# dmiruke/find_motion

Measured on AMD Instinct MI355X. Metric: frames/sec on 1080p synthetic video at 1/2/4/8 MI355X; achieved HBM GB/s %peak, higher is better.
Workload: dtype u8+f64

## Files before the change

### find_motion_amd/csrc/fm_pix.hip

```cpp
#include <type_traits>

#include "fm_internal.h"

namespace fm {
namespace px {

constexpr int TS = 64;
constexpr int kPixWPE = 4;
constexpr int NT = 512;
constexpr int NW = NT / 64;
constexpr int RPWV = TS / NW;

__host__ __device__ constexpr int a16(int v) { return (v + 15) & ~15; }

struct Geo {
    int r, PC, GW, NQ, GH, RS, CPR, nchunks, RSH;
    int o_raw, o_H, o_rowy, o_colx, o_atab, bytes;
    int raw_bytes, H_bytes;
    __host__ __device__ explicit Geo(int rr) {
        r = rr;
        PC = 4 * ((r + 3) / 4);
        GW = TS + 2 * PC;
        NQ = GW / 4;
        GH = TS + 2 * r;
// ... 392 lines not shown
                    uint8_t* gp = a.planes + f * plane + (size_t)y * w;
#pragma unroll
                    for (int b = 0; b < 4; b++)
                        if (xq + b < w) gp[xq + b] = (uint8_t)(g4[it] >> (8 * b));
                }
            }
            uint32_t qv[NQW];
            qv[0] = g4[it];
#pragma unroll
            for (int d = 1; d < NQW; d++)
                qv[d] = d < NQN ? (uint32_t)__builtin_amdgcn_mov_dpp((int)qv[d - 1], 0x130, 0xF, 0xF, true) : 0u;
            {
                const uint32_t h0 = htap<0, OFF, NG, 0, NQW>(qv, cpk, 0u);
                const uint32_t h1 = htap<1, OFF, NG, 0, NQW>(qv, cpk, 0u);
                const uint32_t h2 = htap<2, OFF, NG, 0, NQW>(qv, cpk, 0u);
                const uint32_t h3 = htap<3, OFF, NG, 0, NQW>(qv, cpk, 0u);
                *reinterpret_cast<uint2*>(Hb + hoff[it]) = make_uint2(h0 | (h1 << 16), h2 | (h3 << 16));
            }
        }
    };
    auto stage_raw = [&](const Raw<NCH>& Rr, int buf) __attribute__((always_inline)) { store_raw(Rr, raw + buf * g.raw_bytes, g, tid); };

    const int t0 = a.t_begin, t1 = a.t_end;
    const int skip = __builtin_amdgcn_readfirstlane(a.dbg_skip);
    Raw<NCH> Rw;
    load_raw(Rw, a.src + ((size_t)t0 * S + s) * fbytes, fb32, plan, span);
    stage_raw(Rw, 0);
    if (t0 + 1 < t1) load_raw(Rw, a.src + ((size_t)(t0 + 1) * S + s) * fbytes, fb32, plan, span);
    lds_barrier();
    gray_stage(raw, Hs, (size_t)t0 * S + s);

    auto frame_loop = [&](auto keepc, auto tailc, const ChainCtx ccv) __attribute__((always_inline)) {
        constexpr bool KEEP = decltype(keepc)::value != 0, TAIL = decltype(tailc)::value != 0;
        for (int t = t0; t < t1; t++) {
            const int b = (t - t0) & 1;
            const size_t f = (size_t)t * S + s;
            if (t + 1 < t1) {
                if (!(skip & 8)) stage_raw(Rw, b ^ 1);
                if (t + 2 < t1 && !(skip & 4)) load_raw(Rw, a.src + (f + 2 * S) * fbytes, fb32, plan, span);
            }
            if (!(skip & 16)) lds_barrier();

            uint32_t colbits = 0;
            ChainCtx ccf = ccv;
            ccf.rowvalid = __builtin_amdgcn_readfirstlane(ccf.rowvalid);
            int x0f = __builtin_amdgcn_readfirstlane(x0), y0f = __builtin_amdgcn_readfirstlane(y0), wvf = wv;
            if constexpr (NT == 512) asm volatile("" : "+s"(ccf.colmask), "+s"(ccf.rowvalid), "+s"(x0f), "+s"(y0f), "+s"(wvf));
            asm volatile("" : "+v"(ccf.keep_lo), "+v"(ccf.keep_hi));
            if (!(skip & 2))
                chain_rows<KC, PLANES, INIT, KEEP, TAIL>(a, Hs + b * (g.H_bytes / 2), atab, g, bg, wvf, ln, x0f, y0f, f, ccf,
                                                         init0 && t == t0, colbits);
            reinterpret_cast<uint8_t*>(a.bits)[((f * a.ntiles + ti) * TS + ln) * 8 + wv] = (uint8_t)colbits;

            if (t + 1 < t1 && !(skip & 1))
                gray_stage(raw + (b ^ 1) * g.raw_bytes, Hs + (b ^ 1) * (g.H_bytes / 2), f + S);
        }
    };
    if (!cc.vec) frame_loop(IntC<1>{}, IntC<1>{}, cc);
    else if (cc.hk) frame_loop(IntC<1>{}, IntC<0>{}, cc);
    else frame_loop(IntC<0>{}, IntC<0>{}, cc);

    double* bgo = a.bg_out + (size_t)s * plane;
    const int x = x0 + ln;
#pragma unroll
    for (int j = 0; j < RPWV; j++) {
        const int y = y0 + RPWV * wv + j;
        if (x < w && y < h) bgo[(size_t)y * w + x] = bg[j];
    }
    kstamp_end(a.kstamp);
    if (pts) {
        const uint64_t rt = __builtin_amdgcn_s_memrealtime(), mt = __builtin_amdgcn_s_memtime();
        pts[1] = rt0;
        pts[2] = rt;
        pts[3] = mt - mt0;
    }
}

template <int K> constexpr int tap_c(int t) { return t < 0 || t >= K ? 0 : Taps<K>::c[t]; }
template <int K> constexpr int tap_lo() {
    int i = 0;
    while (Taps<K>::c[i] == 0) i++;
    return i;
}
template <int K> constexpr int tap_hi() {
    int i = K - 1;
    while (Taps<K>::c[i] == 0) i--;
    return i;
}

template <int KC, int RW_ = RPWV>
struct PW {
    static constexpr int NWB = 8;
    static constexpr int RW = RW_;
    static constexpr int R = KC / 2;
    static constexpr int PC = 4 * ((R + 3) / 4);
    static constexpr int NTB = 64 * NWB;
    static constexpr int TH = RW * NWB;
    static constexpr int GH = TH + 2 * R;
    static constexpr int GQ = (TS + 2 * PC) / 4;
    static constexpr int NG = GH * GQ;
    static constexpr int GSLOTS = (NG + 63) / 64;
    static constexpr int gcnt(int w) { return (GSLOTS - w + NWB - 1) / NWB; }
    static constexpr int GJ = gcnt(0);
    static constexpr int NHP = GH / 2;
    static constexpr int NH = NHP * (TS / 4);
    static constexpr int HJ = (NH + NTB - 1) / NTB;
    static constexpr int HLASTW = (NH - (HJ - 1) * NTB + 63) / 64;
#ifndef FM_PIXW_GS
#define FM_PIXW_GS 24
#endif
    static constexpr int GS = FM_PIXW_GS > GQ ? FM_PIXW_GS : GQ;
    static constexpr int GBUF = GH * GS + 64;
    static constexpr int HBUF = (NHP + 1) * TS;
    static constexpr int LO = tap_lo<KC>(), HI = tap_hi<KC>();
    static constexpr int NGR = (HI - LO + 4) / 4;
    static constexpr int OFF = PC - R;
    static constexpr int WQ = (3 + OFF + LO + 4 * NGR - 1) / 4 + 1;
    static constexpr int p0(int j) { return (j + LO) >> 1; }
    static constexpr int np(int j) { return (j + HI + 2 - 2 * p0(j)) / 2; }
    static constexpr int np_max() {
        int m = 0;
        for (int j = 0; j < RW; j++) m = p0(j) + np(j) > m ? p0(j) + np(j) : m;
        return m;
    }
    static constexpr int NP = np_max();
    static constexpr int bytes = 2 * GBUF * 4 + 2 * HBUF * 4 + 256 * 8;
    static constexpr int dyn_bytes = bytes - 256 * 8;
};
template <int KC> constexpr uint32_t tapw4(int g) {
    uint32_t v = 0;
    for (int b = 0; b < 4; b++) {
        const int t = PW<KC>::LO + 4 * g + b;
        if (t <= PW<KC>::HI) v |= (uint32_t)Taps<KC>::c[t] << (8 * b);
    }
    return v;
}
template <int KC> constexpr uint32_t tapv2(int j, int i) {
    const int ft = 2 * (PW<KC>::p0(j) + i) - j;
    return (uint32_t)tap_c<KC>(ft) | (uint32_t)tap_c<KC>(ft + 1) << 16;
}

template <int KC, int RW> constexpr int np_rows() {
    int m = 0;
    for (int j = 0; j < RW; j++) m = PW<KC>::p0(j) + PW<KC>::np(j) > m ? PW<KC>::p0(j) + PW<KC>::np(j) : m;
    return m;
}

template <int RW, int NPR>
__device__ __forceinline__ void chain_pairs(uint32_t (&P)[NPR], const uint32_t* Hp, int wv, int ln) {
    const uint32_t* col = Hp + (RW / 2 * wv) * TS + ln;
#pragma unroll
    for (int i = 0; i < NPR; i++) P[i] = col[i * TS];
}
template <int KC, bool KEEP, bool SDWA, int j, bool H16 = false, int NPR>
__device__ __forceinline__ void chain_blur(const uint32_t (&P)[NPR], const ChainCtx& cc, uint32_t& acc, uint32_t& tix) {
    using G = PW<KC>;
    acc = 32768u;
    static_for<G::np(j)>([&](auto ic) {
        constexpr int i = decltype(ic)::value;
        acc = __builtin_amdgcn_udot2(__builtin_bit_cast(u16x2_t, P[G::p0(j) + i]),
                                     __builtin_bit_cast(u16x2_t, tapv2<KC>(j, i) << (H16 ? 4 : 0)), acc, false);
    });
    if (KEEP) {
        const uint32_t kw = j < 4 ? cc.keep_lo : j < 8 ? cc.keep_hi : j < 12 ? cc.keep_2 : cc.keep_3;
        acc &= (uint32_t)__builtin_amdgcn_sbfe((int)kw, 8 * (j & 3), 8);
    }
    if constexpr (SDWA)
        asm("v_lshlrev_b32_sdwa %0, 3, %1 dst_sel:DWORD dst_unused:UNUSED_PAD src0_sel:DWORD src1_sel:BYTE_2"
            : "=v"(tix) : "v"(acc));
    else
        tix = acc >> 16;
}
template <bool SDWA>
__device__ __forceinline__ double chain_tab(const double* atab, uint32_t tix) {
    return SDWA ? *reinterpret_cast<const double*>(reinterpret_cast<const char*>(atab) + tix) : atab[tix];
}
template <int j>
__device__ __forceinline__ void chain_bit(uint32_t acc, double b, uint32_t bias, uint32_t& tb, uint32_t& tb2) {
    const uint32_t q = __builtin_amdgcn_cvt_pk_u8_f32(fabsf(__double2float_rn(b)), 2, acc);
    const uint32_t r = __builtin_amdgcn_sad_u8(acc, q, bias);
    if constexpr (j < 8) tb = __builtin_amdgcn_udot4(r, (1u << j) << 8, tb, false);
    else tb2 = __builtin_amdgcn_udot4(r, (1u << (j - 8)) << 8, tb2, false);
}
template <bool TAIL, int RW, int j>
__device__ __forceinline__ double chain_bg(const FusedArgs& a, double b, double beta, double bl, int wv, int ln, int x0, int y0,
                                           int w) {
    double nb = bg_fma(b, beta, bl);
    if (TAIL) {
        const long long li = (long long)(y0 + RW * wv + j) * w + x0 + ln;
        if (li >= a.acc_vec_end) nb = __dadd_rn(bl, __dmul_rn(b, beta));
    }
    return nb;
}
template <int RW>
__device__ __forceinline__ void chain_flags(uint32_t tb, uint32_t tb2, const ChainCtx& cc, uint32_t& colbits) {
    if constexpr (RW > 8) tb |= tb2 << 8;
    colbits = tb & cc.tbmask;
    asm volatile("" : "+v"(colbits));
}

template <int KC, bool KEEP, bool TAIL, bool SDWA, int RW = RPWV>
__device__ __forceinline__ void chain_rows_w(const FusedArgs& a, const uint32_t* Hp, const double* atab, double (&bg)[RW],
                                             int wv, int ln, int x0, int y0, const ChainCtx& cc, uint32_t& colbits) {
    static_assert(RW == 8 || RW == 16, "rows per wave");
    uint32_t P[np_rows<KC, RW>()];
    chain_pairs<RW>(P, Hp, wv, ln);
    const int w = a.w;
    const double beta = a.beta;
    const int thr = min(max(a.thresh, -1), 255);
    const uint32_t bias = (uint32_t)(255 - thr);
    uint32_t tb = 0, tb2 = 0;
    static_for<RW>([&](auto jc) {
        constexpr int j = decltype(jc)::value;
        uint32_t acc, tix;
        chain_blur<KC, KEEP, SDWA, j>(P, cc, acc, tix);
        const double b = bg[j];
        chain_bit<j>(acc, b, bias, tb, tb2);
        const double bl = chain_tab<SDWA>(atab, tix);
        bg[j] = chain_bg<TAIL, RW, j>(a, b, beta, bl, wv, ln, x0, y0, w);
    });
    chain_flags<RW>(tb, tb2, cc, colbits);
}

template <int K>
struct HS {
    static constexpr int LO = tap_lo<K>(), NTAPS = tap_hi<K>() - LO + 1, B0 = PW<K>::OFF + LO;
    static constexpr int d0(int k) { return (B0 + k) / 4; }
    static constexpr int nd(int k) { return (B0 + k + NTAPS - 1) / 4 - d0(k) + 1; }
    static constexpr int base(int k) { return k == 0 ? 0 : base(k - 1) + nd(k - 1); }
    static constexpr int NC = base(4);
    static constexpr int NQ = (B0 + 3 + NTAPS - 1) / 4 + 1;
    static constexpr uint32_t c(int k, int i) {
        uint32_t v = 0;
        const int d = d0(k) + i;
        for (int b = 0; b < 4; b++) {
            const int t = 4 * d + b - B0 - k;
            if (t >= 0 && t < NTAPS) v |= (uint32_t)Taps<K>::c[LO + t] << (8 * b);
        }
        return v;
    }
};
template <int K>
__device__ __forceinline__ void hs_consts(uint32_t (&cs)[HS<K>::NC]) {
    static_for<4>([&](auto kc) {
        constexpr int k = decltype(kc)::value;
        static_for<HS<K>::nd(k)>([&](auto ic) {
            constexpr int i = decltype(ic)::value;
            cs[HS<K>::base(k) + i] = HS<K>::c(k, i);
        });
    });
#pragma unroll
    for (int i = 0; i < HS<K>::NC; i++) asm volatile("" : "+v"(cs[i]));
}
template <int K, int k, int N>
__device__ __forceinline__ uint32_t hs_tap(const uint32_t (&q)[N], const uint32_t (&cs)[HS<K>::NC]) {
    static_assert(HS<K>::d0(k) + HS<K>::nd(k) <= N, "window dwords");
    uint32_t acc = 0;
    static_for<HS<K>::nd(k)>([&](auto ic) {
        constexpr int i = decltype(ic)::value;
        acc = __builtin_amdgcn_udot4(q[HS<K>::d0(k) + i], cs[HS<K>::base(k) + i], acc, false);
    });
    return acc;
}

template <int NWB_ = 8>
struct P5G {
    static constexpr int NWB = NWB_;
    static constexpr int RW = TS / NWB;
    static constexpr int NTB = 64 * NWB;
    static constexpr int TH = RW * NWB;
    static constexpr int GH = TH + 4;
    static constexpr int GQ = 18;
#ifndef FM_P5_GS
#define FM_P5_GS 24
#endif
#ifndef FM_P5_GS8
#define FM_P5_GS8 20
#endif
    static constexpr int GS = NWB == 8 ? FM_P5_GS8 : FM_P5_GS > GQ ? FM_P5_GS : GQ;
    static_assert(GS >= 20 && GS % 2 == 0, "a 32-byte window at byte 48 of an 8-byte aligned row");
    static constexpr int NG = GH * GQ;
    static constexpr int GSLOTS = (NG + 63) / 64;
    static constexpr int GFAST = NWB == 8 ? 4 : (GSLOTS + NWB - 1) / NWB;
    static constexpr int GSLOW = NWB == 8 ? (GSLOTS - 4 * GFAST + 3) / 4 : 0;
    static constexpr int GJ = GFAST > GSLOW ? GFAST : GSLOW;
    static constexpr int NH = (GH / 2) * (TS / 4);
    static constexpr int HJ = (NH + NTB - 1) / NTB;
    static constexpr int HLASTW = (NH - (HJ - 1) * NTB + 63) / 64;
    static constexpr int GBUF = GH * GS + 64;
    static constexpr int HBUF = (GH + 2) * TS;
    static constexpr int bytes = 2 * GBUF * 4 + 2 * HBUF * 2 + 256 * 8;
    static constexpr int dyn_bytes = bytes - 256 * 8;
    static constexpr int MROWS = GH / 2, MB = 3;
    static constexpr int moff(int i) { return i == 0 ? 0 : i == 1 ? 16 : MROWS - 16; }
};
static_assert(P5G<8>::MROWS % 2 == 0 && P5G<8>::moff(2) % 2 == 0 && P5G<8>::moff(2) <= 32, "whole row pairs, no gap");
static_assert(P5G<8>::GSLOW >= 0 && 4 * (P5G<8>::GFAST + P5G<8>::GSLOW) >= P5G<8>::GSLOTS, "gray slots");
static_assert(4 * P5G<4>::GFAST >= P5G<4>::GSLOTS, "gray slots");

template <int GJ>
struct P5Raw {
    u32x3_t v[GJ];
};

template <bool KEEP, bool TAIL, int NWB = 8>
__global__ __launch_bounds__(64 * NWB) __attribute__((amdgpu_waves_per_eu(kPixWPE))) void k_pix5(FusedArgs a) {
    using G = P5G<NWB>;
    constexpr int RW = G::RW;
    constexpr int GJX = G::GJ, HJX = G::HJ;
    extern __shared__ __attribute__((aligned(16))) uint8_t smem[];
    constexpr int KC = 5, R = 2;
    uint32_t* gray = reinterpret_cast<uint32_t*>(smem);
    uint16_t* Hs = reinterpret_cast<uint16_t*>(smem + 2 * G::GBUF * 4);
    __shared__ double atab_s[256];
    double* atab = atab_s;
    const int tid = (int)threadIdx.x, ln = tid & 63;
    const int wv = __builtin_amdgcn_readfirstlane(tid >> 6);
    const int s = blockIdx.y;
    const int h = a.h, w = a.w, S = a.S;
    const int ti = swizzle_tile(blockIdx.x, a.ntiles);
    const int tx = ti % a.ntx;
    const int y0 = (ti / a.ntx) * TS;
    const int x0 = tx * TS;
    const size_t plane = (size_t)h * w;
    const size_t fbytes = plane * 3;
    const bool hk = a.has_keep[s] != 0;
    const uint8_t* keep = a.keep + (size_t)s * plane;
    if (tid < 256) atab[tid] = __dmul_rn((double)tid, a.alpha);
    kstamp_begin(a.kstamp);
#ifdef FM_DEV_SWITCHES
    uint64_t* pts = (a.dbg_pts && tid == 0) ? a.dbg_pts + ((size_t)s * a.ntiles + ti) * 4 : nullptr;
    uint64_t rt0 = 0, mt0 = 0;
    if (pts) {
        pts[0] = (uint64_t)__builtin_amdgcn_s_getreg((31 << 11) | 4) | ((uint64_t)__builtin_amdgcn_s_getreg((31 << 11) | 20) << 32);
        rt0 = __builtin_amdgcn_s_memrealtime();
        mt0 = __builtin_amdgcn_s_memtime();
    }
#endif

    uint32_t goff[GJX];
    uint32_t gdst[GJX];
    const int gjobs = NWB == 8 ? (wv < 4 ? G::GFAST : G::GSLOW) : min(G::GFAST, G::GSLOTS - wv * G::GFAST);
#pragma unroll
    for (int i = 0; i < GJX; i++) {
        const int slot = NWB != 8 ? wv * G::GFAST + i : wv >= 4 ? (wv - 4) * G::GSLOW + i : 4 * G::GSLOW + wv * G::GFAST + i;
        const int j = i < gjobs ? slot * 64 + ln : G::NG;
        const int gr = j / G::GQ, gq = j - gr * G::GQ;
        const int x = x0 - 4 + 4 * gq;
        const bool live = j < G::NG && x >= 0 && x + 4 <= w;
        const int y = reflect101(y0 - R + gr, h);
        goff[i] = live ? (uint32_t)(((size_t)y * w + x) * 3) : 0u;
        gdst[i] = j < G::NG ? (uint32_t)(G::GS == G::GQ ? j : gr * G::GS + gq) : (uint32_t)(G::GH * G::GS + ln);
    }
    uint32_t hsrc[HJX], hdst[HJX];
#pragma unroll
    for (int i = 0; i < HJX; i++) {
        const int j = tid + G::NTB * i;
        const bool live = j < G::NH;
        const int hr = live ? j / (TS / 4) : 0, hq = live ? j - hr * (TS / 4) : 0;
        hsrc[i] = (uint32_t)(2 * hr * G::GS + hq);
        hdst[i] = (uint32_t)((live ? hr : G::GH / 2) * TS + 4 * hq);
    }
    const bool edge_tile = x0 == 0 || x0 + TS + 4 > w;
    const int vq = (w - x0 + 4) / 4;
    uint32_t hfix[HJX];
#pragma unroll
    for (int i = 0; i < HJX; i++) {
        const int hq = (int)(hsrc[i] % G::GS);
        hfix[i] = (x0 == 0 && hq == 0 ? 1u : 0u) | (hq + 1 == vq ? 2u : 0u) | (hq + 2 == vq ? 4u : 0u);
    }
    uint32_t asrc = 0, mdst = 0;
    long btap = 0;
    i32x4_t mc0 = {2048, 2048, 2048, 2048};
    if constexpr (NWB == 8) {
        static_assert(Taps<5>::c[0] % 16 == 0 && Taps<5>::c[1] % 16 == 0 && Taps<5>::c[2] % 16 == 0, "taps / 16");
        const int mn = ln & 15, mq = ln >> 4, cb = wv & 3, r0 = (wv >> 2) * G::MROWS;
        asrc = (uint32_t)((r0 + mn) * G::GS * 4 + 16 * cb + 8 * mq);
        mdst = (uint32_t)((r0 / 2 + 2 * mq) * TS + 16 * cb + mn);
        const int bw = w - x0 + 4;
        uint64_t bt = 0;
        static_for<5>([&](auto tc) {
            constexpr int t = decltype(tc)::value;
            int sb = 16 * cb + mn + 2 + t;
            if (x0 == 0 && sb < 4) sb = 8 - sb;
            else if (sb >= bw) sb = 2 * bw - 2 - sb;
            const int k = sb - 16 * cb - 8 * mq;
            bt += (unsigned)k < 8u ? (uint64_t)(Taps<5>::c[t] / 16) << (8 * (k & 7)) : 0ull;
        });
        btap = (long)bt;
        asm volatile("" : "+v"(asrc), "+v"(mdst), "+v"(btap), "+v"(mc0));
    }

    double bg[RW];
    ChainCtx cc;
    auto load_bg = [&]() __attribute__((always_inline)) {
        const double* bgi = a.bg_in + (size_t)s * plane;
        const int x = x0 + ln;
        cc.colmask = __builtin_amdgcn_ballot_w64(x < w);
        cc.rowvalid = 0;
        cc.keep_lo = cc.keep_hi = cc.keep_2 = cc.keep_3 = 0;
        cc.hk = __builtin_amdgcn_readfirstlane(hk ? 1 : 0) != 0;
#pragma unroll
        for (int j = 0; j < RW; j++) {
            const int y = y0 + RW * wv + j;
            const bool in = x < w && y < h;
            if (y < h) cc.rowvalid |= 1u << j;
            bg[j] = in ? bgi[(size_t)y * w + x] : 0.0;
            const uint32_t kb = (!hk || (in && keep[(size_t)y * w + x] != 0)) ? 0xFFu : 0u;
            if (j < 4) cc.keep_lo |= kb << (8 * j);
            else if (j < 8) cc.keep_hi |= kb << (8 * (j - 4));
            else if (j < 12) cc.keep_2 |= kb << (8 * (j - 8));
            else cc.keep_3 |= kb << (8 * (j - 12));
        }
        const long long last = (long long)(y0 + RW * wv + RW - 1) * w + x0 + TS - 1;
        cc.vec = (uint32_t)__builtin_amdgcn_readfirstlane(last < a.acc_vec_end ? 1 : 0);
        cc.tbmask = x < w ? cc.rowvalid : 0u;
#pragma unroll
        for (int j = 0; j < RW; j++) asm volatile("" : "+v"(bg[j]));
        asm volatile("" : "+v"(cc.keep_lo), "+v"(cc.keep_hi));
        if constexpr (RW > 8) asm volatile("" : "+v"(cc.keep_2), "+v"(cc.keep_3));
    };
    if constexpr (NWB != 8) load_bg();

    uint32_t hcs[HS<KC>::NC] = {};
    if constexpr (NWB != 8) hs_consts<KC>(hcs);
    P5Raw<GJX> rw;
    auto load = [&](size_t f) __attribute__((always_inline)) {
        const gbytes_t src = frame_base(a.src + f * fbytes);
#pragma unroll
        for (int i = 0; i < GJX; i++) load12(rw.v[i], src, goff[i]);
    };
    auto gray_stage = [&](uint32_t* gb) __attribute__((always_inline)) {
#pragma unroll
        for (int i = 0; i < GJX; i++) {
            if (i >= gjobs) break;
            gb[gdst[i]] = gray4<NWB == 8>(rw.v[i].x, rw.v[i].y, rw.v[i].z);
        }
    };
    auto mf_read = [&](const uint32_t* gb, auto ic) __attribute__((always_inline)) {
        constexpr int i = decltype(ic)::value;
        return *reinterpret_cast<const long*>(reinterpret_cast<const uint8_t*>(gb) + asrc + G::moff(i) * G::GS * 4);
    };
    auto mf_mul = [&](long av) __attribute__((always_inline)) {
        return __builtin_amdgcn_mfma_i32_16x16x32_i8(av, btap, mc0, 0, 0, 0);
    };
    auto mf_store = [&](uint16_t* Hb, auto ic, i32x4_t d) __attribute__((always_inline)) {
        constexpr int i = decltype(ic)::value;
        uint32_t* hp = reinterpret_cast<uint32_t*>(Hb) + mdst + G::moff(i) / 2 * TS;
        hp[0] = __builtin_amdgcn_perm((uint32_t)d.y, (uint32_t)d.x, 0x05040100u);
        hp[TS] = __builtin_amdgcn_perm((uint32_t)d.w, (uint32_t)d.z, 0x05040100u);
    };
    auto mf_stage = [&](const uint32_t* gb, uint16_t* Hb) __attribute__((always_inline)) {
        static_for<G::MB>([&](auto ic) { mf_store(Hb, ic, mf_mul(mf_read(gb, ic))); });
    };
    auto tap_read = [&](const uint32_t* gb, int i, int row, uint32_t (&q)[3]) __attribute__((always_inline)) {
#pragma unroll
        for (int d = 0; d < 3; d++) q[d] = gb[hsrc[i] + row * G::GS + d];
    };
    auto tap_row = [&](auto edge, int i, const uint32_t (&q)[3], uint32_t (&hh)[4]) __attribute__((always_inline)) {
        uint32_t qv[4] = {q[0], q[1], q[2], 0u};
        if (edge) {
            if (hfix[i] & 1) qv[0] = __builtin_amdgcn_perm(qv[1], qv[1], 0x01020000u);
            if (hfix[i] & 2) qv[1] = __builtin_amdgcn_perm(qv[0], qv[0], 0x00000102u);
            if (hfix[i] & 4) qv[2] = __builtin_amdgcn_perm(qv[1], qv[1], 0x00000102u);
        }
        hh[0] = hs_tap<KC, 0>(qv, hcs);
        hh[1] = hs_tap<KC, 1>(qv, hcs);
        hh[2] = hs_tap<KC, 2>(qv, hcs);
        hh[3] = hs_tap<KC, 3>(qv, hcs);
    };
    auto tap_store = [&](uint16_t* Hb, int i, const uint32_t (&h)[4], const uint32_t (&k)[4]) __attribute__((always_inline)) {
        *reinterpret_cast<uint4*>(reinterpret_cast<uint32_t*>(Hb) + hdst[i]) =
            make_uint4(__builtin_amdgcn_perm(k[0], h[0], 0x05040100u), __builtin_amdgcn_perm(k[1], h[1], 0x05040100u),
                       __builtin_amdgcn_perm(k[2], h[2], 0x05040100u), __builtin_amdgcn_perm(k[3], h[3], 0x05040100u));
    };
    auto tap_job = [&](auto edge, const uint32_t* gb, uint16_t* Hb, int i) __attribute__((always_inline)) {
        uint32_t q[3], h[4], k[4];
        tap_read(gb, i, 0, q);
        tap_row(edge, i, q, h);
        tap_read(gb, i, 1, q);
        tap_row(edge, i, q, k);
        tap_store(Hb, i, h, k);
    };
    auto tap_stage = [&](auto edge, const uint32_t* gb, uint16_t* Hb) __attribute__((always_inline)) {
#pragma unroll
        for (int i = 0; i < HJX; i++) {
            if (i == G::HJ - 1 && wv >= G::HLASTW) break;
            tap_job(edge, gb, Hb, i);
        }
    };
    const int t0 = a.t_begin, t1 = a.t_end;
    auto run = [&](auto edge) __attribute__((always_inline)) {
        if constexpr (NWB == 8) load_bg();
        load((size_t)t0 * S + s);
        gray_stage(gray);
        load((size_t)min(t0 + 1, t1 - 1) * S + s);
        __syncthreads();
        if constexpr (NWB == 8) mf_stage(gray, Hs);
        else tap_stage(edge, gray, Hs);
        if (t0 + 1 < t1) gray_stage(gray + G::GBUF);
        load((size_t)min(t0 + 2, t1 - 1) * S + s);

        const int var0 = TAIL ? (int)(cc.vec == 0) : 0;
        for (int t = t0; t < t1; t++) {
            const int b = (t - t0) & 1;
            const size_t f = (size_t)t * S + s;
            lds_barrier();
            uint32_t colbits = 0;
            ChainCtx ccf = cc;
            ccf.rowvalid = __builtin_amdgcn_readfirstlane(ccf.rowvalid);
            int x0f = __builtin_amdgcn_readfirstlane(x0), y0f = __builtin_amdgcn_readfirstlane(y0), wvf = wv, var = var0;
            asm volatile("" : "+s"(ccf.colmask), "+s"(ccf.rowvalid), "+s"(x0f), "+s"(y0f), "+s"(wvf));
            var = __builtin_amdgcn_readfirstlane(var);
            if constexpr (KEEP) asm volatile("" : "+v"(ccf.keep_lo), "+v"(ccf.keep_hi));
            if constexpr (KEEP && RW > 8) asm volatile("" : "+v"(ccf.keep_2), "+v"(ccf.keep_3));
            const uint32_t* Hp = reinterpret_cast<const uint32_t*>(Hs + b * G::HBUF);
            if constexpr (NWB == 8) {
                const uint32_t* gn = gray + (b ^ 1) * G::GBUF;
                uint16_t* Hn = Hs + (b ^ 1) * G::HBUF;
                static_assert(G::MB == 3 && RW == 8, "three blocks a wave");
                uint32_t P[np_rows<KC, RW>()], acc[4], tb = 0, tb2 = 0;
                double bl[4];
                const double beta = a.beta;
                const uint32_t bias = (uint32_t)(255 - min(max(a.thresh, -1), 255));
                auto blur4 = [&](auto j0) __attribute__((always_inline)) {
                    static_for<4>([&](auto jc) {
                        constexpr int jj = decltype(jc)::value, j = decltype(j0)::value + jj;
                        uint32_t tix;
                        chain_blur<KC, KEEP, true, j, true>(P, ccf, acc[jj], tix);
                        bl[jj] = chain_tab<true>(atab, tix);
                    });
                    __builtin_amdgcn_sched_barrier(0);
                };
                auto rows4 = [&](auto j0, auto tail) __attribute__((always_inline)) {
                    static_for<4>([&](auto jc) {
                        constexpr int jj = decltype(jc)::value, j = decltype(j0)::value + jj;
                        chain_bit<j>(acc[jj], bg[j], bias, tb, tb2);
                        bg[j] = chain_bg<decltype(tail)::value, RW, j>(a, bg[j], beta, bl[jj], wvf, ln, x0f, y0f, w);
                    });
                };
                auto chain4 = [&](auto j0) __attribute__((always_inline)) {
                    if (!TAIL || var == 0) rows4(j0, std::false_type{});
                    else rows4(j0, std::true_type{});
                    __builtin_amdgcn_sched_barrier(0);
                };
                const long a0 = mf_read(gn, IntC<0>{}), a1 = mf_read(gn, IntC<1>{}), a2 = mf_read(gn, IntC<2>{});
                chain_pairs<RW>(P, Hp, wvf, ln);
                __builtin_amdgcn_sched_barrier(0);
                const i32x4_t d0 = mf_mul(a0), d1 = mf_mul(a1), d2 = mf_mul(a2);
                __builtin_amdgcn_sched_barrier(0);
                blur4(std::integral_constant<int, 0>{});
                __builtin_amdgcn_sched_barrier(0);
                chain4(std::integral_constant<int, 0>{});
                blur4(std::integral_constant<int, 4>{});
                mf_store(Hn, IntC<0>{}, d0);
                mf_store(Hn, IntC<1>{}, d1);
                mf_store(Hn, IntC<2>{}, d2);
                __builtin_amdgcn_sched_barrier(0);
                chain4(std::integral_constant<int, 4>{});
                chain_flags<RW>(tb, tb2, ccf, colbits);
            } else {
                if (!TAIL || var == 0)
                    chain_rows_w<KC, KEEP, false, true, RW>(a, Hp, atab, bg, wvf, ln, x0f, y0f, ccf, colbits);
                else
                    chain_rows_w<KC, KEEP, true, true, RW>(a, Hp, atab, bg, wvf, ln, x0f, y0f, ccf, colbits);
                if (t + 1 < t1) tap_stage(edge, gray + (b ^ 1) * G::GBUF, Hs + (b ^ 1) * G::HBUF);
            }
            gray_stage(gray + b * G::GBUF);
            if constexpr (RW == 8)
                reinterpret_cast<uint8_t*>(a.bits)[((f * a.ntiles + ti) * TS + ln) * 8 + wv] = (uint8_t)colbits;
            else
                reinterpret_cast<uint16_t*>(a.bits)[((f * a.ntiles + ti) * TS + ln) * 4 + wv] = (uint16_t)colbits;
            load((size_t)min(t + 3, t1 - 1) * S + s);
        }
    };
    if constexpr (NWB == 8) run(std::false_type{});
    else run(edge_tile);

    double* bgo = a.bg_out + (size_t)s * plane;
    const int x = x0 + ln;
#pragma unroll
    for (int j = 0; j < RW; j++) {
        const int y = y0 + RW * wv + j;
        if (x < w && y < h) bgo[(size_t)y * w + x] = bg[j];
    }
    kstamp_end(a.kstamp);
#ifdef FM_DEV_SWITCHES
    if (pts) {
        const uint64_t rt = __builtin_amdgcn_s_memrealtime(), mt = __builtin_amdgcn_s_memtime();
        pts[1] = rt0;
        pts[2] = rt;
        pts[3] = mt - mt0;
    }
#endif
}

#ifndef FM_PIXW_WPE
#define FM_PIXW_WPE kPixWPE
#endif
template <int KC, bool KEEP, bool TAIL, int RW = RPWV>
__global__ __launch_bounds__(512) __attribute__((amdgpu_waves_per_eu(RW == 16 ? FM_PIXW_WPE : kPixWPE))) void k_pixw(FusedArgs a) {
    using G = PW<KC, RW>;
    constexpr int TPB = RW / RPWV;
    constexpr int GJX = G::GJ, HJX = G::HJ;
    extern __shared__ __attribute__((aligned(16))) uint8_t smem[];
    constexpr int R = G::R, PC = G::PC, GQ = G::GQ;
    uint32_t* gray = reinterpret_cast<uint32_t*>(smem);
    uint32_t* Hs = reinterpret_cast<uint32_t*>(smem + 2 * G::GBUF * 4);
    __shared__ double atab_s[256];
    double* atab = atab_s;
    const int tid = threadIdx.x, ln = tid & 63;
    const int wv = __builtin_amdgcn_readfirstlane(tid >> 6);
    const int s = blockIdx.y;
    const int h = a.h, w = a.w, S = a.S;
    const int bi = swizzle_tile(blockIdx.x, TPB == 1 ? a.ntiles : a.ntx * ((a.nty + TPB - 1) / TPB));
    const int tx = bi % a.ntx;
    const int y0 = (bi / a.ntx) * G::TH;
    const int x0 = tx * TS;
    const int tyw = (bi / a.ntx) * TPB + (TPB == 1 ? 0 : (wv >> 2));
    const bool tile_ok = TPB == 1 || tyw < a.nty;
    const int ti = TPB == 1 ? bi : tyw * a.ntx + tx;
    const size_t plane = (size_t)h * w;
    const size_t fbytes = plane * 3;
    const bool hk = a.has_keep[s] != 0;
    const uint8_t* keep = a.keep + (size_t)s * plane;
    if (tid < 256) atab[tid] = __dmul_rn((double)tid, a.alpha);
    kstamp_begin(a.kstamp);

    const int gcnt_w = G::gcnt(wv);
    auto gplan = [&](int i, int lnv, uint32_t& go, uint32_t& gd) __attribute__((always_inline)) {
        const int slot = i * G::NWB + wv;
        const int j = (i < gcnt_w && slot < G::GSLOTS) ? slot * 64 + lnv : G::NG;
        const int gr = j / GQ, gq = j - gr * GQ;
        const int x = x0 - PC + 4 * gq;
        const bool live = j < G::NG && x >= 0 && x + 4 <= w;
        const int y = reflect101(y0 - R + gr, h);
        go = live ? (uint32_t)(((size_t)y * w + x) * 3) : 0u;
        gd = j < G::NG ? (uint32_t)(gr * G::GS + gq) : (uint32_t)(G::GH * G::GS + lnv);
    };
    auto hplan = [&](int i, int tidv, uint32_t& hs, uint32_t& hd, int& hq_) __attribute__((always_inline)) {
        const int j = tidv + G::NTB * i;
        const bool live = j < G::NH;
        const int hp = live ? j / (TS / 4) : 0, hq = live ? j - hp * (TS / 4) : 0;
        hq_ = hq;
        hs = (uint32_t)(2 * hp * G::GS + hq);
        hd = (uint32_t)((live ? hp : G::NHP) * TS + 4 * hq);
    };
    uint32_t goff[GJX], gdst[GJX], hsrc[HJX], hdst[HJX];
    int hqv[HJX];
#pragma unroll
    for (int i = 0; i < GJX; i++) gplan(i, ln, goff[i], gdst[i]);
#pragma unroll
    for (int i = 0; i < HJX; i++) hplan(i, tid, hsrc[i], hdst[i], hqv[i]);
    const int gjobs = __builtin_amdgcn_readfirstlane(gcnt_w);
    const bool edge_tile = x0 - PC < 0 || x0 + TS + PC > w;

    double bg[RW];
    ChainCtx cc;
    {
        const double* bgi = a.bg_in + (size_t)s * plane;
        const int x = x0 + ln;
        cc.colmask = __builtin_amdgcn_ballot_w64(x < w);
        cc.rowvalid = 0;
        cc.keep_lo = cc.keep_hi = cc.keep_2 = cc.keep_3 = 0;
        cc.hk = __builtin_amdgcn_readfirstlane(hk ? 1 : 0) != 0;
#pragma unroll
        for (int j = 0; j < RW; j++) {
            const int y = y0 + RW * wv + j;
            const bool in = x < w && y < h;
            if (y < h) cc.rowvalid |= 1u << j;
            bg[j] = in ? bgi[(size_t)y * w + x] : 0.0;
            const uint32_t kb = (!hk || (in && keep[(size_t)y * w + x] != 0)) ? 0xFFu : 0u;
            if (j < 4) cc.keep_lo |= kb << (8 * j);
            else if (j < 8) cc.keep_hi |= kb << (8 * (j - 4));
            else if (j < 12) cc.keep_2 |= kb << (8 * (j - 8));
            else cc.keep_3 |= kb << (8 * (j - 12));
        }
        const long long last = (long long)(y0 + RW * wv + RW - 1) * w + x0 + TS - 1;
        cc.vec = (uint32_t)__builtin_amdgcn_readfirstlane(last < a.acc_vec_end ? 1 : 0);
        cc.tbmask = x < w ? cc.rowvalid : 0u;
    }
#pragma unroll
    for (int j = 0; j < RW; j++) asm volatile("" : "+v"(bg[j]));
    asm volatile("" : "+v"(cc.keep_lo), "+v"(cc.keep_hi));
    if constexpr (RW > 8) asm volatile("" : "+v"(cc.keep_2), "+v"(cc.keep_3));

    uint32_t cpk[G::NGR];
#pragma unroll
    for (int gi = 0; gi < G::NGR; gi++) cpk[gi] = tapw4<KC>(gi);
    u32x3_t rw[GJX];
    auto load = [&](size_t f) __attribute__((always_inline)) {
        const __amdgpu_buffer_rsrc_t rs = frame_rsrc(a.src + f * fbytes, (uint32_t)fbytes);
#pragma unroll
        for (int i = 0; i < GJX; i++) load12b(rw[i], rs, goff[i]);
    };
    auto gray_stage = [&](uint32_t* gb) __attribute__((always_inline)) {
#pragma unroll
        for (int i = 0; i < GJX; i++) {
            if (i >= gjobs) break;
            gb[gdst[i]] = gray4(rw[i].x, rw[i].y, rw[i].z);
        }
    };
    auto hrow = [&](const uint32_t* row, int hq, uint32_t (&o)[4]) __attribute__((always_inline)) {
        uint32_t qv[G::WQ];
#pragma unroll
        for (int d = 0; d < G::WQ; d++) qv[d] = row[hq + d];
        if (edge_tile) {
            int hqe = hq, xe = x0 - PC;
            asm volatile("" : "+v"(hqe), "+v"(xe));
#pragma unroll
            for (int d = 0; d < G::WQ; d++) {
                const int c = xe + 4 * (hqe + d);
                if (c < 0 || c >= w) {
                    const int sp = c < 0 ? -(c + 3) : 2 * w - 5 - c;
                    const int qa = min(max((sp - (x0 - PC)) >> 2, 0), GQ - 2);
                    qv[d] = __builtin_amdgcn_perm(row[qa + 1], row[qa], c < 0 ? 0x01020304u : 0x03040506u);
                }
            }
        }
        o[0] = htap<0, G::OFF + G::LO, G::NGR, 0, G::WQ>(qv, cpk, 0u);
        o[1] = htap<1, G::OFF + G::LO, G::NGR, 0, G::WQ>(qv, cpk, 0u);
        o[2] = htap<2, G::OFF + G::LO, G::NGR, 0, G::WQ>(qv, cpk, 0u);
        o[3] = htap<3, G::OFF + G::LO, G::NGR, 0, G::WQ>(qv, cpk, 0u);
    };
    auto tap_stage = [&](const uint32_t* gb, uint32_t* Hb) __attribute__((always_inline)) {
#pragma unroll
        for (int i = 0; i < HJX; i++) {
            if (i == G::HJ - 1 && wv >= G::HLASTW) break;
            const uint32_t hs = hsrc[i], hd = hdst[i];
            const int hq = hqv[i];
            const uint32_t* r0 = gb + (hs - hq);
            uint32_t u[4], v[4];
            hrow(r0, hq, u);
            hrow(r0 + G::GS, hq, v);
            *reinterpret_cast<uint4*>(Hb + hd) = make_uint4(u[0] | (v[0] << 16), u[1] | (v[1] << 16),
                                                             u[2] | (v[2] << 16), u[3] | (v[3] << 16));
// ... 145 lines not shown
```

Measured before the change: 493,600.

## Compute full 5x5 blur with MFMA 16x16x64 and drop the LDS horizontal buffer

The NWB=8 path previously used an MFMA for the horizontal blur pass, staged results into an LDS H buffer, then did the vertical pass with udot2 chains. It now folds both passes into two chained i8 16x16x64 MFMAs per block, using separable tap products packed into the B operands, so the blurred values come straight from the accumulator registers. This removes the H buffer's LDS traffic and storage, remaps each lane's pixel ownership to the MFMA output layout (bg load/store, bit packing via permlane16_swap, new bits indexing), and lowers GFAST to 3. The cost is more complex operand addressing, extra gray reads per block, and a risk of precision or layout mismatches in the fused tap encoding.

```diff
diff --git a/find_motion_amd/csrc/fm_pix.hip b/find_motion_amd/csrc/fm_pix.hip
--- a/find_motion_amd/csrc/fm_pix.hip
+++ b/find_motion_amd/csrc/fm_pix.hip
@@ -568,14 +568,14 @@
 #pragma unroll
     for (int i = 0; i < NPR; i++) P[i] = col[i * TS];
 }
-template <int KC, bool KEEP, bool SDWA, int j, bool H16 = false, int NPR>
+template <int KC, bool KEEP, bool SDWA, int j, int NPR>
 __device__ __forceinline__ void chain_blur(const uint32_t (&P)[NPR], const ChainCtx& cc, uint32_t& acc, uint32_t& tix) {
     using G = PW<KC>;
     acc = 32768u;
     static_for<G::np(j)>([&](auto ic) {
         constexpr int i = decltype(ic)::value;
         acc = __builtin_amdgcn_udot2(__builtin_bit_cast(u16x2_t, P[G::p0(j) + i]),
-                                     __builtin_bit_cast(u16x2_t, tapv2<KC>(j, i) << (H16 ? 4 : 0)), acc, false);
+                                     __builtin_bit_cast(u16x2_t, tapv2<KC>(j, i)), acc, false);
     });
     if (KEEP) {
         const uint32_t kw = j < 4 ? cc.keep_lo : j < 8 ? cc.keep_hi : j < 12 ? cc.keep_2 : cc.keep_3;
@@ -591,9 +591,9 @@
 __device__ __forceinline__ double chain_tab(const double* atab, uint32_t tix) {
     return SDWA ? *reinterpret_cast<const double*>(reinterpret_cast<const char*>(atab) + tix) : atab[tix];
 }
-template <int j>
+template <int j, int BYTE = 2>
 __device__ __forceinline__ void chain_bit(uint32_t acc, double b, uint32_t bias, uint32_t& tb, uint32_t& tb2) {
-    const uint32_t q = __builtin_amdgcn_cvt_pk_u8_f32(fabsf(__double2float_rn(b)), 2, acc);
+    const uint32_t q = __builtin_amdgcn_cvt_pk_u8_f32(fabsf(__double2float_rn(b)), BYTE, acc);
     const uint32_t r = __builtin_amdgcn_sad_u8(acc, q, bias);
     if constexpr (j < 8) tb = __builtin_amdgcn_udot4(r, (1u << j) << 8, tb, false);
     else tb2 = __builtin_amdgcn_udot4(r, (1u << (j - 8)) << 8, tb2, false);
@@ -697,7 +697,10 @@
     static_assert(GS >= 20 && GS % 2 == 0, "a 32-byte window at byte 48 of an 8-byte aligned row");
     static constexpr int NG = GH * GQ;
     static constexpr int GSLOTS = (NG + 63) / 64;
-    static constexpr int GFAST = NWB == 8 ? 4 : (GSLOTS + NWB - 1) / NWB;
+#ifndef FM_P5_GFAST
+#define FM_P5_GFAST 3
+#endif
+    static constexpr int GFAST = NWB == 8 ? FM_P5_GFAST : (GSLOTS + NWB - 1) / NWB;
     static constexpr int GSLOW = NWB == 8 ? (GSLOTS - 4 * GFAST + 3) / 4 : 0;
     static constexpr int GJ = GFAST > GSLOW ? GFAST : GSLOW;
     static constexpr int NH = (GH / 2) * (TS / 4);
@@ -705,12 +708,13 @@
     static constexpr int HLASTW = (NH - (HJ - 1) * NTB + 63) / 64;
     static constexpr int GBUF = GH * GS + 64;
     static constexpr int HBUF = (GH + 2) * TS;
-    static constexpr int bytes = 2 * GBUF * 4 + 2 * HBUF * 2 + 256 * 8;
+    static constexpr int bytes = 2 * GBUF * 4 + (NWB == 8 ? 0 : 2 * HBUF * 2) + 256 * 8;
     static constexpr int dyn_bytes = bytes - 256 * 8;
-    static constexpr int MROWS = GH / 2, MB = 3;
-    static constexpr int moff(int i) { return i == 0 ? 0 : i == 1 ? 16 : MROWS - 16; }
+    static constexpr int MROWS = 32, MB = 2;
+    static constexpr int moff(int i) { return 16 * i; }
 };
-static_assert(P5G<8>::MROWS % 2 == 0 && P5G<8>::moff(2) % 2 == 0 && P5G<8>::moff(2) <= 32, "whole row pairs, no gap");
+static_assert(2 * P5G<8>::MROWS == P5G<8>::TH && P5G<8>::MROWS + P5G<8>::moff(1) + 15 + 4 < P5G<8>::GH, "operand rows in the gray buffer");
+static_assert(P5G<8>::GS % 4 == 0 && P5G<8>::GS * 4 >= 48 + 24, "16-byte aligned rows that hold the last block's 24-byte window");
 static_assert(P5G<8>::GSLOW >= 0 && 4 * (P5G<8>::GFAST + P5G<8>::GSLOW) >= P5G<8>::GSLOTS, "gray slots");
 static_assert(4 * P5G<4>::GFAST >= P5G<4>::GSLOTS, "gray slots");
 
@@ -785,30 +789,72 @@
         const int hq = (int)(hsrc[i] % G::GS);
         hfix[i] = (x0 == 0 && hq == 0 ? 1u : 0u) | (hq + 1 == vq ? 2u : 0u) | (hq + 2 == vq ? 4u : 0u);
     }
-    uint32_t asrc = 0, mdst = 0;
-    long btap = 0;
-    i32x4_t mc0 = {2048, 2048, 2048, 2048};
+    uint32_t asrc = 0, asrc2 = 0, asrc3 = 0, asrc2b = 0, asrc3b = 0, bdst = 0;
+    long long li0 = 0;
+    i32x4_t btap1 = {0, 0, 0, 0}, btap2 = {0, 0, 0, 0};
+    i32x4_t mc0 = {32896, 32896, 32896, 32896};
     if constexpr (NWB == 8) {
         static_assert(Taps<5>::c[0] % 16 == 0 && Taps<5>::c[1] % 16 == 0 && Taps<5>::c[2] % 16 == 0, "taps / 16");
         const int mn = ln & 15, mq = ln >> 4, cb = wv & 3, r0 = (wv >> 2) * G::MROWS;
-        asrc = (uint32_t)((r0 + mn) * G::GS * 4 + 16 * cb + 8 * mq);
-        mdst = (uint32_t)((r0 / 2 + 2 * mq) * TS + 16 * cb + mn);
+        const int s2 = 2 * mq, s3 = 2 * mq + 1;
+        asrc = (uint32_t)((r0 + mn + mq) * G::GS * 4 + 16 * cb);
+        asrc2 = (uint32_t)((r0 + mn + (s2 < 2 ? 4 : s2 - 2)) * G::GS * 4 + 16 * cb + (s2 < 2 ? 8 * s2 : 16));
+        asrc3 = (uint32_t)((r0 + mn + (s3 < 2 ? 4 : min(s3 - 2, 4))) * G::GS * 4 + 16 * cb + (s3 < 2 ? 8 * s3 : 16));
         const int bw = w - x0 + 4;
-        uint64_t bt = 0;
+        uint64_t hw0 = 0, hw1 = 0, hw2 = 0;
         static_for<5>([&](auto tc) {
             constexpr int t = decltype(tc)::value;
             int sb = 16 * cb + mn + 2 + t;
             if (x0 == 0 && sb < 4) sb = 8 - sb;
             else if (sb >= bw) sb = 2 * bw - 2 - sb;
-            const int k = sb - 16 * cb - 8 * mq;
-            bt += (unsigned)k < 8u ? (uint64_t)(Taps<5>::c[t] / 16) << (8 * (k & 7)) : 0ull;
+            const int k = sb - 16 * cb;
+            const uint64_t v = (uint64_t)(Taps<5>::c[t] / 16) << (8 * (k & 7));
+            hw0 += (unsigned)k < 8u ? v : 0ull;
+            hw1 += (unsigned)(k - 8) < 8u ? v : 0ull;
+            hw2 += (unsigned)(k - 16) < 8u ? v : 0ull;
         });
-        btap = (long)bt;
-        asm volatile("" : "+v"(asrc), "+v"(mdst), "+v"(btap), "+v"(mc0));
+        auto cv = [](int dr) { return (uint64_t)(dr == 0 || dr == 4 ? Taps<5>::c[0] / 16 : dr == 2 ? Taps<5>::c[2] / 16 : Taps<5>::c[1] / 16); };
+        static_assert(Taps<5>::c[0] == Taps<5>::c[4] && Taps<5>::c[1] == Taps<5>::c[3], "symmetric taps");
+        const uint64_t b1l = hw0 * cv(mq), b1h = hw1 * cv(mq);
+        const uint64_t b2l = mq == 0 ? hw0 * cv(4) : hw2 * cv(s2 - 2);
+        const uint64_t b2h = mq == 0 ? hw1 * cv(4) : mq == 3 ? 0ull : hw2 * cv(s3 - 2);
+        btap1 = i32x4_t{(int)(uint32_t)b1l, (int)(uint32_t)(b1l >> 32), (int)(uint32_t)b1h, (int)(uint32_t)(b1h >> 32)};
+        btap2 = i32x4_t{(int)(uint32_t)b2l, (int)(uint32_t)(b2l >> 32), (int)(uint32_t)b2h, (int)(uint32_t)(b2h >> 32)};
+        const int bi = 4 * (wv >> 2) + 2 * (mq & 1) + (mq >> 1);
+        bdst = (uint32_t)((16 * cb + mn) * 8 + bi);
+        asrc2b = asrc2 + G::moff(1) * G::GS * 4;
+        asrc3b = asrc3 + G::moff(1) * G::GS * 4;
+        asm volatile("" : "+v"(asrc), "+v"(asrc2), "+v"(asrc3), "+v"(asrc2b), "+v"(asrc3b), "+v"(bdst), "+v"(btap1), "+v"(btap2), "+v"(mc0));
     }
 
     double bg[RW];
     ChainCtx cc;
+    auto load_bg8 = [&]() __attribute__((always_inline)) {
+        const double* bgi = a.bg_in + (size_t)s * plane;
+        const int mn = ln & 15, mq = ln >> 4, cb = wv & 3;
+        const int x = x0 + 16 * cb + mn, yl = y0 + G::MROWS * (wv >> 2) + 4 * mq;
+        cc.colmask = 0;
+        cc.rowvalid = 0;
+        cc.keep_lo = cc.keep_hi = cc.keep_2 = cc.keep_3 = 0;
+        cc.hk = __builtin_amdgcn_readfirstlane(hk ? 1 : 0) != 0;
+#pragma unroll
+        for (int j = 0; j < RW; j++) {
+            const int y = yl + G::moff(j >> 2) + (j & 3);
+            const bool in = x < w && y < h;
+            bg[j] = in ? bgi[(size_t)y * w + x] : 0.0;
+            const uint32_t kb = (!hk || (in && keep[(size_t)y * w + x] != 0)) ? 0xFFu : 0u;
+            if (j < 4) cc.keep_lo |= kb << (8 * j);
+            else cc.keep_hi |= kb << (8 * (j - 4));
+        }
+        const int yb = y0 + 8 * (int)(bdst & 7);
+        cc.tbmask = x < w ? (yb + 8 <= h ? 0xFFu : yb < h ? (1u << (h - yb)) - 1u : 0u) : 0u;
+        li0 = (long long)yl * w + x;
+        const long long last = (long long)(y0 + G::MROWS * (wv >> 2) + G::MROWS - 1) * w + x0 + 16 * cb + 15;
+        cc.vec = (uint32_t)__builtin_amdgcn_readfirstlane(last < a.acc_vec_end ? 1 : 0);
+#pragma unroll
+        for (int j = 0; j < RW; j++) asm volatile("" : "+v"(bg[j]));
+        asm volatile("" : "+v"(cc.keep_lo), "+v"(cc.keep_hi));
+    };
     auto load_bg = [&]() __attribute__((always_inline)) {
         const double* bgi = a.bg_in + (size_t)s * plane;
         const int x = x0 + ln;
@@ -853,21 +899,20 @@
             gb[gdst[i]] = gray4<NWB == 8>(rw.v[i].x, rw.v[i].y, rw.v[i].z);
         }
     };
-    auto mf_read = [&](const uint32_t* gb, auto ic) __attribute__((always_inline)) {
+    auto mf_read = [&](const uint32_t* gb, auto ic, i32x4_t& a1, i32x4_t& a2) __attribute__((always_inline)) {
         constexpr int i = decltype(ic)::value;
-        return *reinterpret_cast<const long*>(reinterpret_cast<const uint8_t*>(gb) + asrc + G::moff(i) * G::GS * 4);
-    };
-    auto mf_mul = [&](long av) __attribute__((always_inline)) {
-        return __builtin_amdgcn_mfma_i32_16x16x32_i8(av, btap, mc0, 0, 0, 0);
-    };
-    auto mf_store = [&](uint16_t* Hb, auto ic, i32x4_t d) __attribute__((always_inline)) {
-        constexpr int i = decltype(ic)::value;
-        uint32_t* hp = reinterpret_cast<uint32_t*>(Hb) + mdst + G::moff(i) / 2 * TS;
-        hp[0] = __builtin_amdgcn_perm((uint32_t)d.y, (uint32_t)d.x, 0x05040100u);
-        hp[TS] = __builtin_amdgcn_perm((uint32_t)d.w, (uint32_t)d.z, 0x05040100u);
-    };
-    auto mf_stage = [&](const uint32_t* gb, uint16_t* Hb) __attribute__((always_inline)) {
-        static_for<G::MB>([&](auto ic) { mf_store(Hb, ic, mf_mul(mf_read(gb, ic))); });
+        const uint8_t* g8 = reinterpret_cast<const uint8_t*>(gb);
+        a1 = *reinterpret_cast<const i32x4_t*>(g8 + asrc + G::moff(i) * G::GS * 4);
+        const uint2 lo = *reinterpret_cast<const uint2*>(g8 + (i == 0 ? asrc2 : asrc2b));
+        const uint2 hi = *reinterpret_cast<const uint2*>(g8 + (i == 0 ? asrc3 : asrc3b));
+        a2 = i32x4_t{(int)lo.x, (int)lo.y, (int)hi.x, (int)hi.y};
+    };
+    auto mf_mul2 = [&](i32x4_t (&d)[2], const i32x4_t& a01, const i32x4_t& a02, const i32x4_t& a11, const i32x4_t& a12)
+        __attribute__((always_inline)) {
+        const i32x4_t e0 = __builtin_amdgcn_mfma_i32_16x16x64_i8(a01, btap1, mc0, 0, 0, 0);
+        const i32x4_t e1 = __builtin_amdgcn_mfma_i32_16x16x64_i8(a11, btap1, mc0, 0, 0, 0);
+        d[0] = __builtin_amdgcn_mfma_i32_16x16x64_i8(a02, btap2, e0, 0, 0, 0);
+        d[1] = __builtin_amdgcn_mfma_i32_16x16x64_i8(a12, btap2, e1, 0, 0, 0);
     };
     auto tap_read = [&](const uint32_t* gb, int i, int row, uint32_t (&q)[3]) __attribute__((always_inline)) {
 #pragma unroll
@@ -907,13 +952,20 @@
     };
     const int t0 = a.t_begin, t1 = a.t_end;
     auto run = [&](auto edge) __attribute__((always_inline)) {
-        if constexpr (NWB == 8) load_bg();
+        if constexpr (NWB == 8) load_bg8();
         load((size_t)t0 * S + s);
         gray_stage(gray);
         load((size_t)min(t0 + 1, t1 - 1) * S + s);
         __syncthreads();
-        if constexpr (NWB == 8) mf_stage(gray, Hs);
-        else tap_stage(edge, gray, Hs);
+        i32x4_t dblk[2] = {mc0, mc0};
+        if constexpr (NWB == 8) {
+            i32x4_t a01, a02, a11, a12;
+            mf_read(gray, IntC<0>{}, a01, a02);
+            mf_read(gray, IntC<1>{}, a11, a12);
+            mf_mul2(dblk, a01, a02, a11, a12);
+        } else {
+            tap_stage(edge, gray, Hs);
+        }
         if (t0 + 1 < t1) gray_stage(gray + G::GBUF);
         load((size_t)min(t0 + 2, t1 - 1) * S + s);
 
@@ -930,52 +982,58 @@
             var = __builtin_amdgcn_readfirstlane(var);
             if constexpr (KEEP) asm volatile("" : "+v"(ccf.keep_lo), "+v"(ccf.keep_hi));
             if constexpr (KEEP && RW > 8) asm volatile("" : "+v"(ccf.keep_2), "+v"(ccf.keep_3));
-            const uint32_t* Hp = reinterpret_cast<const uint32_t*>(Hs + b * G::HBUF);
             if constexpr (NWB == 8) {
                 const uint32_t* gn = gray + (b ^ 1) * G::GBUF;
-                uint16_t* Hn = Hs + (b ^ 1) * G::HBUF;
-                static_assert(G::MB == 3 && RW == 8, "three blocks a wave");
-                uint32_t P[np_rows<KC, RW>()], acc[4], tb = 0, tb2 = 0;
+                static_assert(G::MB == 2 && RW == 8, "two blocks a wave");
+                uint32_t acc[4], tb = 0, tb2 = 0;
                 double bl[4];
                 const double beta = a.beta;
                 const uint32_t bias = (uint32_t)(255 - min(max(a.thresh, -1), 255));
-                auto blur4 = [&](auto j0) __attribute__((always_inline)) {
+                auto blur4 = [&](auto ic) __attribute__((always_inline)) {
+                    constexpr int i = decltype(ic)::value;
                     static_for<4>([&](auto jc) {
-                        constexpr int jj = decltype(jc)::value, j = decltype(j0)::value + jj;
+                        constexpr int jj = decltype(jc)::value;
+                        acc[jj] = (uint32_t)dblk[i][jj];
+                        if (KEEP) acc[jj] &= (uint32_t)__builtin_amdgcn_sbfe((int)(i == 0 ? ccf.keep_lo : ccf.keep_hi), 8 * jj, 8);
                         uint32_t tix;
-                        chain_blur<KC, KEEP, true, j, true>(P, ccf, acc[jj], tix);
+                        asm("v_lshlrev_b32_sdwa %0, 3, %1 dst_sel:DWORD dst_unused:UNUSED_PAD src0_sel:DWORD src1_sel:BYTE_1"
+                            : "=v"(tix) : "v"(acc[jj]));
                         bl[jj] = chain_tab<true>(atab, tix);
                     });
                     __builtin_amdgcn_sched_barrier(0);
                 };
-                auto rows4 = [&](auto j0, auto tail) __attribute__((always_inline)) {
+                auto rows4 = [&](auto ic, auto tail) __attribute__((always_inline)) {
+                    constexpr int i = decltype(ic)::value;
                     static_for<4>([&](auto jc) {
-                        constexpr int jj = decltype(jc)::value, j = decltype(j0)::value + jj;
-                        chain_bit<j>(acc[jj], bg[j], bias, tb, tb2);
-                        bg[j] = chain_bg<decltype(tail)::value, RW, j>(a, bg[j], beta, bl[jj], wvf, ln, x0f, y0f, w);
+                        constexpr int jj = decltype(jc)::value, j = 4 * i + jj;
+                        chain_bit<8 * i + jj, 1>(acc[jj], bg[j], bias, tb, tb2);
+                        double nb = bg_fma(bg[j], beta, bl[jj]);
+                        if constexpr (decltype(tail)::value) {
+                            if (li0 + (long long)(G::moff(i) + jj) * w >= a.acc_vec_end) nb = __dadd_rn(bl[jj], __dmul_rn(bg[j], beta));
+                        }
+                        bg[j] = nb;
                     });
                 };
-                auto chain4 = [&](auto j0) __attribute__((always_inline)) {
-                    if (!TAIL || var == 0) rows4(j0, std::false_type{});
-                    else rows4(j0, std::true_type{});
+                auto chain4 = [&](auto ic) __attribute__((always_inline)) {
+                    if (!TAIL || var == 0) rows4(ic, std::false_type{});
+                    else rows4(ic, std::true_type{});
                     __builtin_amdgcn_sched_barrier(0);
                 };
-                const long a0 = mf_read(gn, IntC<0>{}), a1 = mf_read(gn, IntC<1>{}), a2 = mf_read(gn, IntC<2>{});
-                chain_pairs<RW>(P, Hp, wvf, ln);
+                i32x4_t a01, a02, a11, a12;
+                mf_read(gn, IntC<0>{}, a01, a02);
+                mf_read(gn, IntC<1>{}, a11, a12);
                 __builtin_amdgcn_sched_barrier(0);
-                const i32x4_t d0 = mf_mul(a0), d1 = mf_mul(a1), d2 = mf_mul(a2);
+                blur4(IntC<0>{});
+                chain4(IntC<0>{});
+                blur4(IntC<1>{});
+                chain4(IntC<1>{});
+                mf_mul2(dblk, a01, a02, a11, a12);
+                const auto sw = __builtin_amdgcn_permlane16_swap(tb, tb2, false, false);
+                colbits = (sw[0] | sw[1] << 4) & ccf.tbmask;
+                asm volatile("" : "+v"(colbits));
                 __builtin_amdgcn_sched_barrier(0);
-                blur4(std::integral_constant<int, 0>{});
-                __builtin_amdgcn_sched_barrier(0);
-                chain4(std::integral_constant<int, 0>{});
-                blur4(std::integral_constant<int, 4>{});
-                mf_store(Hn, IntC<0>{}, d0);
-                mf_store(Hn, IntC<1>{}, d1);
-                mf_store(Hn, IntC<2>{}, d2);
-                __builtin_amdgcn_sched_barrier(0);
-                chain4(std::integral_constant<int, 4>{});
-                chain_flags<RW>(tb, tb2, ccf, colbits);
             } else {
+                const uint32_t* Hp = reinterpret_cast<const uint32_t*>(Hs + b * G::HBUF);
                 if (!TAIL || var == 0)
                     chain_rows_w<KC, KEEP, false, true, RW>(a, Hp, atab, bg, wvf, ln, x0f, y0f, ccf, colbits);
                 else
@@ -984,7 +1042,7 @@
             }
             gray_stage(gray + b * G::GBUF);
             if constexpr (RW == 8)
-                reinterpret_cast<uint8_t*>(a.bits)[((f * a.ntiles + ti) * TS + ln) * 8 + wv] = (uint8_t)colbits;
+                reinterpret_cast<uint8_t*>(a.bits)[(f * a.ntiles + ti) * TS * 8 + bdst] = (uint8_t)colbits;
             else
                 reinterpret_cast<uint16_t*>(a.bits)[((f * a.ntiles + ti) * TS + ln) * 4 + wv] = (uint16_t)colbits;
             load((size_t)min(t + 3, t1 - 1) * S + s);
@@ -994,10 +1052,10 @@
     else run(edge_tile);
 
     double* bgo = a.bg_out + (size_t)s * plane;
-    const int x = x0 + ln;
+    const int x = NWB == 8 ? x0 + 16 * (wv & 3) + (ln & 15) : x0 + ln;
 #pragma unroll
     for (int j = 0; j < RW; j++) {
-        const int y = y0 + RW * wv + j;
+        const int y = NWB == 8 ? y0 + G::MROWS * (wv >> 2) + 4 * (ln >> 4) + G::moff(j >> 2) + (j & 3) : y0 + RW * wv + j;
         if (x < w && y < h) bgo[(size_t)y * w + x] = bg[j];
     }
     kstamp_end(a.kstamp);
```

Result: faster. 499,400, median of 6 (+1.2%).
